# ArmastusChen/Learning-Continuous-Implicit-Representation-for-Near-Periodic-Patterns

Hardware: AMD Instinct MI355X
Metric: fitted pixels/sec/GPU (512^2 grid, 256-wide MLP) + iters-to-target-PSNR (higher is better)
Workload: dtype bf16

## Files before the change

### learning-continuous-implicit-representation-for-near-periodic-patterns_amd/csrc/npp_api.hip

```cpp
#include <math.h>
#include <stdarg.h>
#include <stdio.h>
#include <string.h>
#include <vector>

#include "npp_adam.h"
#include "npp_chain16.h"
#include "npp_stash_census.h"

namespace npp {

static thread_local char g_err[512] = "";

void set_error(const char* fmt, ...) {
  va_list ap;
  va_start(ap, fmt);
  vsnprintf(g_err, sizeof(g_err), fmt, ap);
  va_end(ap);
}

int check_launch(const char* what) {
  hipError_t e = hipGetLastError();
  if (e != hipSuccess) {
    set_error("%s: %s", what, hipGetErrorString(e));
// ... 165 lines not shown
#pragma unroll
  for (int e = 0; e < 4; ++e) {
    if (e < cnt) {
      if (n < d.n_out[l]) {
        const __bf16 w = (__bf16)pn[e];
        if (!fwd4) {
          const int64_t pf = fwd_pack_pos(d, l, n, k);
          if (pf >= 0) a.wf[pf] = w;
        }
        const int64_t pb = bwd_pack_pos(b, l, n, k);
        if (pb >= 0) a.wb[pb] = w;
      }
      if (++k == d.n_in[l]) { k = 0; ++n; }
      if (n >= d.n_out[l] && i + e + 1 >= d.b_off[l] + d.n_out[l]) {
        do { ++l; } while (l < kNumLayers && !d.present[l]);
        if (l >= kNumLayers) break;
        n = 0; k = 0;
      }
    }
  }
}

static uint16_t f32_to_bf16_host(float f) {
  uint32_t u;
  memcpy(&u, &f, 4);
  if ((u & 0x7fffffffu) > 0x7f800000u) return (uint16_t)((u >> 16) | 0x40);
  u += 0x7FFF + ((u >> 16) & 1);
  return (uint16_t)(u >> 16);
}

__global__ void selftest_kernel(float* out) {
  const int lane = threadIdx.x & 63;
  const int m = lane & 31, h = lane >> 5;
  bf16x8 a, b;
#pragma unroll
  for (int j = 0; j < 8; ++j) {
    const int k = 8 * h + j;
    a[j] = (__bf16)(float)(((m * 3 + k * 5) % 5) - 2);
    b[j] = (__bf16)(float)(((k * 7 + m * 2) % 4) - 1);
  }
  f32x16 acc = {};
  acc = mfma_bf16(a, b, acc);
#pragma unroll
  for (int r = 0; r < 16; ++r) out[acc_row(r, h) * 32 + m] = acc[r];
  f32x16 y = {};
#pragma unroll
  for (int s = 0; s < 2; ++s) {
    bf16x8 x = pack_acc(acc, s), a2;
#pragma unroll
    for (int j = 0; j < 8; ++j) {
      const int k = 16 * s + perm16(h, j);
      a2[j] = (__bf16)(float)(((m * 5 + k * 3) % 7) - 3);
    }
    y = mfma_bf16(a2, x, y);
  }
#pragma unroll
  for (int r = 0; r < 16; ++r) out[1024 + acc_row(r, h) * 32 + m] = y[r];

  __shared__ __attribute__((aligned(16))) char tile[16384];
  for (int u = lane; u < 1024; u += 64) {
    const int hh = u & 1, b = (u >> 1) & 31, bt = (u >> 6) & 1, ks = u >> 7;
    bf16x8 f;
#pragma unroll
    for (int j = 0; j < 8; ++j) {
      const int feat = 16 * ks + perm16(hh, j), row = bt * 32 + b;
      f[j] = (__bf16)(float)(((7 * feat + 3 * row) % 251) - 125);
    }
    *(bf16x8*)(tile + wfmt_unit(8, 0, ks, bt, b, hh)) = f;
  }
  __syncthreads();
  for (int tt = 0; tt < 4; ++tt)
    for (int t = 0; t < 4; ++t) {
      const bf16x8 f = wfrag_read(tile, wfrag_offset(tt, t, lane));
#pragma unroll
      for (int j = 0; j < 8; ++j) out[2048 + ((tt * 4 + t) * 64 + lane) * 8 + j] = (float)f[j];
    }
}

static int tune_env(const char* name, int dflt) {
  const char* e = getenv(name);
  return e && *e ? atoi(e) : dflt;
}
Tunables g_tune = {tune_env("NPP_CONV_WINK", 1), tune_env("NPP_CONV_WIN", 1), tune_env("NPP_CONV_WSTAT", 1), tune_env("NPP_CONV_PAIR", 15),
                   tune_env("NPP_LIGHT_DET", 1), tune_env("NPP_STASH8", 1)};

}

using namespace npp;

extern "C" {

int npp_version(void) { return 100; }

int npp_tune(const char* key, int value) {
  struct { const char* k; int* v; } tab[] = {{"conv_wink", &g_tune.conv_wink}, {"conv_win", &g_tune.conv_win},
                                             {"conv_wstat", &g_tune.conv_wstat}, {"conv_pair", &g_tune.conv_pair},
                                             {"stash8", &g_tune.stash8}, {"light_det", &g_tune.light_det}};
  if (key)
    for (auto& t : tab)
      if (!strcmp(key, t.k)) {
        const int old = __atomic_load_n(t.v, __ATOMIC_RELAXED);
        if (value >= 0) __atomic_store_n(t.v, value, __ATOMIC_RELAXED);
        return old;
      }
  set_error("npp_tune: unknown key '%s'", key ? key : "(null)");
  return NPP_ERR_ARG;
}
const char* npp_last_error_string(void) { return g_err; }

int npp_device_count(void) {
  int n = 0;
  hipError_t e = hipGetDeviceCount(&n);
  if (e != hipSuccess) {
    set_error("hipGetDeviceCount: %s", hipGetErrorString(e));
    (void)hipGetLastError();
    return 0;
  }
  return n;
}

static int check_kw(int K, int width) {
  if (K < 1 || K > NPP_MAX_K) { set_error("K=%d outside [1,%d]", K, NPP_MAX_K); return NPP_ERR_ARG; }
  if (width != NPP_WIDTH) {
    set_error("width=%d: this build is specialised for width %d", width, NPP_WIDTH);
    return NPP_ERR_UNSUPPORTED;
  }
  return NPP_OK;
}

int npp_param_layout(int K, int width, const char** names, int64_t* offsets, int32_t* rows,
                     int32_t* cols, int64_t* total) {
  int rc = check_kw(K, width);
  if (rc) return rc;
  const NetDesc d = make_desc(K);
  int n = 0;
  for (int l = 0; l < kNumLayers; ++l) {
    if (!d.present[l]) continue;
    for (int wb = 0; wb < 2; ++wb) {
      snprintf(g_name_buf[n], sizeof(g_name_buf[n]), "%s.%s", kNames[l], wb ? "bias" : "weight");
      if (names) names[n] = g_name_buf[n];
      if (offsets) offsets[n] = wb ? d.b_off[l] : d.w_off[l];
      if (rows) rows[n] = d.n_out[l];
      if (cols) cols[n] = wb ? 1 : d.n_in[l];
      ++n;
    }
  }
  if (total) *total = d.total_params;
  return n;
}

int64_t npp_pack_bytes(int K, int width, int which) {
  if (check_kw(K, width)) return -1;
  return 16 * (which == 0 ? make_desc(K).wf_total16 : bwd_total16(K));
}

int npp_pack_weights(const float* d_params, void* d_wf, void* d_wb, int K, int width, void* stream) {
  int rc = check_kw(K, width);
  if (rc) return rc;
  if (!d_params || !d_wf || !d_wb) { set_error("npp_pack_weights: null pointer"); return NPP_ERR_ARG; }
  const NetDesc d = make_desc(K);
  const BwdDesc b = make_bwd_desc(K);
  const int64_t nf = d.wf_total16, nb = bwd_total16(K);
  const int threads = 256;
  const int64_t blocks = (nf + nb + threads - 1) / threads;
  hipLaunchKernelGGL(pack_weights_kernel, dim3((unsigned)blocks), dim3(threads), 0, (hipStream_t)stream,
                     d_params, (bf16x8*)d_wf, (bf16x8*)d_wb, d, b, nf, nb);
  return check_launch("npp_pack_weights");
}

int npp_pack_weights_host(const float* params, void* wf, void* wb, int K, int width) {
  int rc = check_kw(K, width);
  if (rc) return rc;
  const NetDesc d = make_desc(K);
  const BwdDesc b = make_bwd_desc(K);
  uint16_t* f = (uint16_t*)wf;
  uint16_t* g = (uint16_t*)wb;
  for (int64_t u = 0; u < d.wf_total16; ++u) {
    int l, ks, nt, lane;
    if (!fwd_unit(d, u, l, ks, nt, lane)) { set_error("fwd unit %lld unmapped", (long long)u); return NPP_ERR_ARG; }
    for (int j = 0; j < 8; ++j) f[u * 8 + j] = f32_to_bf16_host(fwd_pack_value(params, d, l, ks, nt, lane, j));
// ... 242 lines not shown
```

### learning-continuous-implicit-representation-for-near-periodic-patterns_amd/csrc/npp_common.h

```cpp
#pragma once
#include <hip/hip_runtime.h>
#include <math.h>
#include <stdint.h>
#include "npp_layout.h"

typedef __attribute__((ext_vector_type(8))) __bf16 bf16x8;
typedef __attribute__((ext_vector_type(4))) __bf16 bf16x4;
typedef __attribute__((ext_vector_type(2))) __bf16 bf16x2;
typedef __attribute__((ext_vector_type(16))) float f32x16;
typedef __attribute__((ext_vector_type(4))) float f32x4;
typedef __attribute__((ext_vector_type(2))) float f32x2;
typedef __attribute__((ext_vector_type(4))) uint32_t u32x4;
typedef __attribute__((ext_vector_type(8))) _Float16 f16x8;

namespace npp {

void set_error(const char* fmt, ...);
int check_launch(const char* what);
struct SmemOnce { unsigned long long done = 0; };
bool smem_attr(SmemOnce& once, const void* fn, int bytes);

constexpr int kLdsDefault = 48 * 1024;
template <auto Kern, typename... Args>
int launch_lds(const char* who, dim3 grid, dim3 block, size_t lds_bytes, int lds_limit, hipStream_t stream, const Args&... args) {
  static SmemOnce once;
  if (lds_limit && !smem_attr(once, (const void*)Kern, lds_limit)) { set_error("%s: smem attribute", who); return NPP_ERR_LAUNCH; }
  hipLaunchKernelGGL(Kern, grid, block, lds_bytes, stream, args...);
  return check_launch(who);
}

struct Tunables {
  int conv_wink;
  int conv_win;
  int conv_wstat;
  int conv_pair;
  int light_det;
  int stash8;
};
extern Tunables g_tune;

constexpr float kInv2Pi = 0.15915494309189535f;

__device__ __forceinline__ float snake_fast(float z) {
  const float s = __builtin_amdgcn_sinf(z * kInv2Pi);
  return fmaf(s, s, z);
}
__device__ __forceinline__ void snake_fast2(float z, float& a, float& da) {
  const float rev = z * kInv2Pi;
  const float s = __builtin_amdgcn_sinf(rev);
  const float c = __builtin_amdgcn_cosf(rev);
  a = fmaf(s, s, z);
  da = fmaf(2.0f * s, c, 1.0f);
}

__device__ __forceinline__ void wg_barrier() {
  asm volatile("s_waitcnt lgkmcnt(0)" ::: "memory");
  __builtin_amdgcn_s_barrier();
  asm volatile("" ::: "memory");
}

using wrsrc_t = __amdgpu_buffer_rsrc_t;
__device__ __forceinline__ wrsrc_t make_wrsrc(const void* pack, int64_t units16) {
  return __builtin_amdgcn_make_buffer_rsrc(const_cast<void*>(pack), 0, (int)(units16 * 16), 0x00020000);
}

struct StackIter {
  int32_t active, k, comp, with_lp;
  int32_t x0, nk, same, pad1;
  float step_size, inv_sqrt_bc2, pad2, pad3;
};
static_assert(sizeof(StackIter) == 48, "npp_stack_iter layout");
struct Stack {
  int32_t M;
  int32_t g;
  int32_t n_items;
  int32_t pad;
  const StackIter* iter;
};
inline Stack make_stack(int M, int n_items, const void* d_iter) {
  Stack S{};
  S.M = M; S.n_items = n_items; S.iter = (const StackIter*)d_iter;
  S.g = (M == 1 || M == 2 || M == 4 || M == 8) ? 8 / M : 0;
  return S;
}
inline unsigned stack_grid(const Stack& S) {
  return S.g ? 8u * (unsigned)((S.n_items + S.g - 1) / S.g) : (unsigned)S.M * (unsigned)S.n_items;
}
__device__ __forceinline__ bool stack_decode(const Stack& S, int& img, int& item, int& xslot, int& xcount) {
  const int b = (int)blockIdx.x;
  if (S.M == 0) { img = 0; item = b; xslot = b >> 3; xcount = ((int)gridDim.x + 7) >> 3; return true; }
  if (S.g) {
    const int xcd = b & 7, slot = b >> 3;
    img = xcd / S.g;
    item = slot * S.g + xcd % S.g;
    xslot = slot; xcount = (S.n_items + S.g - 1) / S.g;
  } else {
    img = b / S.n_items;
    item = b - img * S.n_items;
    xslot = item >> 3; xcount = (S.n_items + 7) >> 3;
  }
  if (item >= S.n_items) return false;
  return S.iter == nullptr || S.iter[img].active != 0;
}

}
```

### learning-continuous-implicit-representation-for-near-periodic-patterns_amd/csrc/npp_cx.hip

```cpp
#include <stdlib.h>

#include "npp_robust.h"
#include <type_traits>
#include "npp_trunk_layout.h"

namespace npp {

__global__ void patch_gather_kernel(const float* __restrict__ img, const float* __restrict__ mask, int H, int W,
                                    const int32_t* __restrict__ centres, int M, int P, float* __restrict__ out_rgb,
                                    float* __restrict__ out_mask) {
  const int m = blockIdx.y;
  const int cy = centres[2 * m], cx = centres[2 * m + 1];
  for (int idx = blockIdx.x * blockDim.x + threadIdx.x; idx < P * P; idx += gridDim.x * blockDim.x) {
    const int py = idx / P, px = idx - py * P;
    const int y = cy - P / 2 + py, x = cx - P / 2 + px;
    const bool in = y >= 0 && y < H && x >= 0 && x < W;
    const int64_t src = (int64_t)y * W + x;
#pragma unroll
    for (int c = 0; c < 3; ++c) out_rgb[((int64_t)m * 3 + c) * P * P + idx] = in ? img[src * 3 + c] : 0.0f;
    if (out_mask) out_mask[(int64_t)m * P * P + idx] = in ? mask[src] : 0.0f;
  }
}

struct CxWs {
  float* mu;
  float* ssx;
  float* ssy;
  unsigned* dmin;
  float* s;
  unsigned* cmax;
  float* dot;
  float* g;
  float* lsum;
  unsigned* ticket;
  float* inx;
  float* iny;
  float* D;
  float* cx;
  const StackIter* iter;
  int32_t M, mu_stride, N, dot_slots;
  int32_t min_in_rows;
};
__device__ __forceinline__ int cx_group(const CxWs& w, int n, int& ng) {
  if (!w.iter) { ng = w.N; return 0; }
  int m = 0;
  for (int j = 1; j < w.M; ++j)
    if (w.iter[j].nk > 0 && n >= w.iter[j].x0) m = j;
  ng = w.iter[m].nk;
  return m;
}
__device__ __forceinline__ const float* cx_mu(const CxWs& w, int n) {
  int ng;
  return w.mu + (int64_t)cx_group(w, n, ng) * w.mu_stride;
}

__host__ __device__ inline int64_t cx_ws_floats(int N, int C, int hw) {
  return (int64_t)NPP_MAX_STACK * (C + 16) + (7LL + C / 32) * N * hw + 3LL * N + 2LL * N * hw * hw + 160;
}

__host__ inline CxWs carve(float* base, int N, int C, int hw, const void* iter = nullptr, int M = 0) {
  CxWs w;
  float* p = base;
  w.iter = (const StackIter*)iter; w.M = M; w.N = N; w.mu_stride = (C + 15) / 16 * 16; w.dot_slots = C / 32; w.min_in_rows = 0;
  w.mu = p; p += (int64_t)(M > 0 ? M : 1) * w.mu_stride;
  const int64_t nh = (int64_t)N * hw;
  w.ssx = p; p += nh;
  w.ssy = p; p += nh;
  w.dmin = (unsigned*)p; p += nh;
  w.s = p; p += nh;
  w.cmax = (unsigned*)p; p += nh;
  w.dot = p; p += nh * w.dot_slots;
  w.g = p; p += (N + 15) / 16 * 16;
  w.lsum = p; p += (N + 15) / 16 * 16;
  w.ticket = (unsigned*)p; p += (N + 1 + 15) / 16 * 16;
  w.inx = p; p += nh;
  w.iny = p; p += nh;
  w.D = p; p += nh * hw;
  w.cx = p;
  return w;
}

__device__ __forceinline__ float inv_norm(float ss) { return 1.0f / fmaxf(sqrtf(ss), 1e-12f); }

// ... 408 lines not shown
  }
}

constexpr int kBigR = 8;
__global__ __launch_bounds__(256) void cx_colmax_big_kernel(int N, int hw, float inv_h, CxWs w, const float* __restrict__ s4) {
  __shared__ float red[4][128];
  const int wave = threadIdx.x >> 6, lane = threadIdx.x & 63;
  const int tiles = (hw + 127) / 128;
  int b = blockIdx.x;
  const int rg = b % kBigR; b /= kBigR;
  const int tj = b % tiles, n = b / tiles;
  if (n >= N) return;
  const int tr = (tiles + kBigR - 1) / kBigR;
  float best0 = 0.0f, best1 = 0.0f;
  for (int ti = rg * tr; ti < min(tiles, (rg + 1) * tr); ++ti) {
    const float* Dt = w.D + (((int64_t)n * tiles + ti) * tiles + tj) * 16384 + wave * 128 + 2 * lane;
    const int irow = ti * 128 + wave + 4 * (lane & 31);
    float my_rdm = 0.0f, my_rs = 0.0f;
    if (irow < hw) {
      const int64_t row = (int64_t)n * hw + irow;
      my_rdm = 1.0f / (__uint_as_float(w.dmin[row]) + 1e-5f);
      const float* sq = s4 + row * kBigQ;
      my_rs = 1.0f / (((sq[0] + sq[1]) + sq[2]) + sq[3]);
    }
#pragma unroll
    for (int k = 0; k < 32; ++k) {
      const float2 d = *(const float2*)(Dt + k * 512);
      const float rdm = __shfl(my_rdm, k, 64), rs = __shfl(my_rs, k, 64);
      const float c0 = __expf((1.0f - d.x * rdm) * inv_h) * rs, c1 = __expf((1.0f - d.y * rdm) * inv_h) * rs;
      best0 = fmaxf(best0, rs > 0.0f ? c0 : 0.0f);
      best1 = fmaxf(best1, rs > 0.0f ? c1 : 0.0f);
    }
  }
  red[wave][2 * lane] = best0;
  red[wave][2 * lane + 1] = best1;
  __syncthreads();
  if (threadIdx.x < 128) {
    const int j = tj * 128 + threadIdx.x;
    const float v = fmaxf(fmaxf(red[0][threadIdx.x], red[1][threadIdx.x]), fmaxf(red[2][threadIdx.x], red[3][threadIdx.x]));
    if (j < hw) atomicMax(&w.cmax[(int64_t)n * hw + j], __float_as_uint(v));
  }
}

__global__ void cx_loss_kernel(int N, int hw, const float* __restrict__ weight, float scale, float* __restrict__ loss,
                               int loss_stride, CxWs w) {
  __shared__ float red[4];
  const int n = blockIdx.x;
  int ng;
  cx_group(w, n, ng);
  float acc = 0.0f;
  for (int j = threadIdx.x; j < hw; j += blockDim.x) {
    acc += __uint_as_float(w.cmax[(int64_t)n * hw + j]);
    w.inx[(int64_t)n * hw + j] = inv_norm(w.ssx[(int64_t)n * hw + j]);
    w.iny[(int64_t)n * hw + j] = inv_norm(w.ssy[(int64_t)n * hw + j]);
  }
  for (int off = 32; off > 0; off >>= 1) acc += __shfl_xor(acc, off, 64);
  if ((threadIdx.x & 63) == 0) red[threadIdx.x >> 6] = acc;
  __syncthreads();
  if (threadIdx.x == 0) {
    const float cxn = (red[0] + red[1] + red[2] + red[3]) / (float)hw;
    float l, dcxn;
    if (weight) {
      const float wt = weight[n];
      l = -logf(cxn * wt + 1e-5f);
      dcxn = -wt / (cxn * wt + 1e-5f);
    } else {
      l = -logf(cxn + 1e-5f) / (float)ng;
      dcxn = -1.0f / ((float)ng * (cxn + 1e-5f));
    }
    share_store(w.lsum + n, scale * l);
    w.g[n] = scale * dcxn / (float)hw;
  }
  if (!block_last_arriver(w.ticket, N)) return;
  const int groups = w.iter ? w.M : 1;
  if ((int)threadIdx.x < groups) {
    const int grp = threadIdx.x;
    const int n0 = w.iter ? w.iter[grp].x0 : 0, cnt = w.iter ? w.iter[grp].nk : N;
    float total = 0.0f;
    for (int q = n0; q < n0 + cnt; ++q) total += share_load(w.lsum + q);
    if (cnt > 0) atomicAdd(loss + (int64_t)grp * loss_stride, total);
  }
}

__global__ __launch_bounds__(256) void cx_rows_bwd_kernel(int N, int hw, float inv_h, CxWs w, float* __restrict__ loss, int loss_stride) {
  const int wave = threadIdx.x >> 6, lane = threadIdx.x & 63;
  if (loss && blockIdx.x == 0 && (int)threadIdx.x < (w.iter ? w.M : 1)) {
    const int grp = threadIdx.x;
    const int n0 = w.iter ? w.iter[grp].x0 : 0, cnt = w.iter ? w.iter[grp].nk : N;
    float total = 0.0f;
    for (int q = n0; q < n0 + cnt; ++q) total += w.lsum[q];
    if (cnt > 0) atomicAdd(loss + (int64_t)grp * loss_stride, total);
  }
  const int64_t row = (int64_t)blockIdx.x * 4 + wave;
  if (row >= (int64_t)N * hw) return;
  const int n = (int)(row / hw);
  const float dmv = __uint_as_float(w.dmin[row]);
  const float dm = dmv + 1e-5f;
  const float s = w.s[row], g = w.g[n];
  const float* Dr = w.D + row * hw;
  float* cr = w.cx + row * hw;
  const unsigned* cm = w.cmax + (int64_t)n * hw;
  float A = 0.0f;
  for (int j = lane; j < hw; j += 64) {
    const float c = cr[j];
    if (__float_as_uint(c) == cm[j]) A += g * c;
  }
  for (int off = 32; off > 0; off >>= 1) A += __shfl_xor(A, off, 64);
  float corr = 0.0f;
  int jmin = 0x7fffffff;
  for (int j = lane; j < hw; j += 64) {
    const float c = cr[j], d = Dr[j];
    const float G = (__float_as_uint(c) == cm[j]) ? g : 0.0f;
    const float wv = c * s;
    const float dDt = -((G - A) / s) * wv * inv_h;
    corr += dDt * d;
    const float dD = dDt / dm;
    cr[j] = (d > 0.0f && d < 1.0f) ? -dD : 0.0f;
    if (d == dmv) jmin = min(jmin, j);
  }
  for (int off = 32; off > 0; off >>= 1) {
    corr += __shfl_xor(corr, off, 64);
    jmin = min(jmin, __shfl_xor(jmin, off, 64));
  }
  if (jmin < hw && lane == (jmin & 63)) {
    const float d = Dr[jmin];
    if (d > 0.0f && d < 1.0f) cr[jmin] += corr / (dm * dm);
  }
}

__global__ __launch_bounds__(256) void cx_dx_kernel(const float* __restrict__ x, const float* __restrict__ y, int N, int C,
                                                    int hw, CxWs w, float* __restrict__ dxh) {
  __shared__ float sA[2][kCxKc][65];
  __shared__ float sB[2][kCxKc][65];
  const int tid = threadIdx.x, wave = tid >> 6, lane = tid & 63;
  const int itiles = (hw + 63) / 64, ctiles = (C + 63) / 64;
  const int n = blockIdx.x / (ctiles * itiles);
  const int rem = blockIdx.x - n * ctiles * itiles;
  const int c0 = (rem / itiles) * 64, i0 = (rem % itiles) * 64;
  const int wc = wave >> 1, wi = wave & 1, l31 = lane & 31, kh = lane >> 5;
  const bool vec = (hw & 3) == 0;
  const float* iny_ss = w.ssy + (int64_t)n * hw;
  const float* mup = cx_mu(w, n);
  float4 ra[2], rb[2];
  auto gload = [&](int j0) {
#pragma unroll
    for (int r = 0; r < 2; ++r) {
      const int idx = tid + 256 * r, row = idx >> 3, col = (idx & 7) * 4;
      const int j = j0 + col;
      float va[4] = {0, 0, 0, 0}, vb[4] = {0, 0, 0, 0};
      const int c = c0 + row, i = i0 + row;
      if (c < C) {
        const float m = mup[c];
        const float* yr = y + ((int64_t)n * C + c) * hw;
        if (vec && j + 3 < hw) { const float4 q = *(const float4*)(yr + j); va[0] = q.x - m; va[1] = q.y - m; va[2] = q.z - m; va[3] = q.w - m; }
        else for (int e = 0; e < 4; ++e) if (j + e < hw) va[e] = yr[j + e] - m;
        for (int e = 0; e < 4; ++e) va[e] = (j + e < hw) ? va[e] * inv_norm(iny_ss[j + e]) : 0.0f;
      }
      if (i < hw) {
        const float* dr = w.cx + ((int64_t)n * hw + i) * hw;
        if (vec && j + 3 < hw) { const float4 q = *(const float4*)(dr + j); vb[0] = q.x; vb[1] = q.y; vb[2] = q.z; vb[3] = q.w; }
        else for (int e = 0; e < 4; ++e) if (j + e < hw) vb[e] = dr[j + e];
      }
      ra[r] = make_float4(va[0], va[1], va[2], va[3]);
      rb[r] = make_float4(vb[0], vb[1], vb[2], vb[3]);
    }
  };
  auto sstore = [&](int buf) {
#pragma unroll
    for (int r = 0; r < 2; ++r) {
      const int idx = tid + 256 * r, row = idx >> 3, col = (idx & 7) * 4;
      sA[buf][col + 0][row] = ra[r].x; sA[buf][col + 1][row] = ra[r].y; sA[buf][col + 2][row] = ra[r].z; sA[buf][col + 3][row] = ra[r].w;
      sB[buf][col + 0][row] = rb[r].x; sB[buf][col + 1][row] = rb[r].y; sB[buf][col + 2][row] = rb[r].z; sB[buf][col + 3][row] = rb[r].w;
    }
  };
  f32x16 acc;
#pragma unroll
  for (int r = 0; r < 16; ++r) acc[r] = 0.0f;
  gload(0);
  sstore(0);
  __syncthreads();
  int buf = 0;
  for (int j0 = 0; j0 < hw; j0 += kCxKc) {
    const bool has_next = j0 + kCxKc < hw;
    if (has_next) gload(j0 + kCxKc);
#pragma unroll
    for (int ks = 0; ks < kCxKc / 2; ++ks) {
      const float a = sA[buf][2 * ks + kh][wc * 32 + l31];
      const float b = sB[buf][2 * ks + kh][wi * 32 + l31];
      acc = __builtin_amdgcn_mfma_f32_32x32x2f32(a, b, acc, 0, 0, 0);
    }
    if (has_next) sstore(buf ^ 1);
    __syncthreads();
    buf ^= 1;
  }
  const int i = i0 + wi * 32 + l31;
  float part = 0.0f;
  if (i < hw) {
    const float inx = inv_norm(w.ssx[(int64_t)n * hw + i]);
#pragma unroll
    for (int r = 0; r < 16; ++r) {
      const int c = c0 + wc * 32 + acc_row(r, kh);
      if (c < C) {
        const int64_t o = ((int64_t)n * C + c) * hw + i;
        dxh[o] = acc[r];
        part = fmaf((x[o] - mup[c]) * inx, acc[r], part);
      }
    }
  }
  part += __shfl_xor(part, 32, 64);
  const int slot = c0 / 32 + wc;
  if (kh == 0 && i < hw && slot < w.dot_slots) w.dot[(int64_t)slot * N * hw + (int64_t)n * hw + i] = part;
}

__global__ void cx_dx_finish_kernel(const float* __restrict__ x, int N, int C, int hw, CxWs w, float* __restrict__ dx, int n_dot) {
  const int64_t t = (int64_t)blockIdx.x * blockDim.x + threadIdx.x;
  if (t >= (int64_t)N * C * hw) return;
  const int p = (int)(t % hw);
  const int64_t nc = t / hw;
  const int c = (int)(nc % C), n = (int)(nc / C);
  const float inx = inv_norm(w.ssx[(int64_t)n * hw + p]);
  float dot = 0.0f;
  for (int q = 0; q < n_dot; ++q) dot += w.dot[(int64_t)q * N * hw + (int64_t)n * hw + p];
  dx[t] = (dx[t] - (x[t] - cx_mu(w, n)[c]) * inx * dot) * inx;
}

__global__ void cx_dx_finish_flat_kernel(const float* __restrict__ x, const float* __restrict__ dxh, int N, int N_total, int C, int H,
                                         int W, CxWs w, const f16x8* __restrict__ yact, bf16x8* __restrict__ dz, int64_t nposp,
                                         int64_t npos_range, int n_dot) {
  const int64_t t = (int64_t)blockIdx.x * blockDim.x + threadIdx.x;
  const int chunks = C / 8;
  if (t >= npos_range * chunks) return;
  const int c8 = (int)(t / npos_range);
  const int64_t p = t - (int64_t)c8 * npos_range;
  const int Wp = W + 2, S = (H + 2) * Wp, hw = H * W;
  const int n = (int)(p / S), r = (int)(p - (int64_t)n * S), yy = r / Wp, xx = r - yy * Wp;
  if (n >= N && n < N_total) return;
  const int64_t u = (int64_t)c8 * nposp + kConvGuard + p;
  bf16x8 o;
#pragma unroll
  for (int j = 0; j < 8; ++j) o[j] = (__bf16)0.0f;
  if (n < N && yy >= 1 && yy <= H && xx >= 1 && xx <= W) {
    const int pos = (yy - 1) * W + (xx - 1);
    const int64_t np = (int64_t)n * hw + pos;
    const float inx = inv_norm(w.ssx[np]);
    float dot = 0.0f;
    for (int q = 0; q < n_dot; ++q) dot += w.dot[(int64_t)q * N * hw + np];
    const float* mu = cx_mu(w, n);
    const f16x8 m = yact[u];
#pragma unroll
    for (int j = 0; j < 8; ++j) {
      const int c = conv_chan(c8, j);
      const int64_t e = ((int64_t)n * C + c) * hw + pos;
      const float v = (dxh[e] - (x[e] - mu[c]) * inx * dot) * inx;
      o[j] = (__bf16)((float)m[j] > 0.0f ? v : 0.0f);
    }
  }
  dz[u] = o;
}


constexpr int kDxLd = 33;
__global__ __launch_bounds__(256) void cx_dx32s_kernel(const float* __restrict__ x, const float* __restrict__ y, int N, int C,
                                                       int hw, CxWs w, float* __restrict__ dxh) {
  __shared__ float sY[2][4][32][kDxLd];
  __shared__ float sD[2][32][kDxLd];
  const int tid = threadIdx.x, wave = tid >> 6, lane = tid & 63, l31 = lane & 31, kh = lane >> 5;
  const int t32 = hw / 32, ct = C / 32, cg = ct / 4 + (ct % 4 ? 1 : 0);
  const int lb = xcd_block(N * t32 * cg);
  if (lb < 0) return;
  const int n = lb / (t32 * cg);
  const int rem = lb - n * t32 * cg;
  const int ti = rem / cg, tc0 = (rem - ti * cg) * 4, tc = tc0 + wave;
  const int i0 = ti * 32, c0 = tc * 32;
  const float* mup = cx_mu(w, n);
  const int srow = tid >> 3, scol = tid & 7;
  const float4* dsrc = (const float4*)(w.cx + ((int64_t)n * hw + i0 + srow) * hw) + scol;
  const float4* ssrc = (const float4*)(w.iny + (int64_t)n * hw) + scol;
  const float4* ysrc[4];
  float mus[4];
#pragma unroll
  for (int q = 0; q < 4; ++q) {
    const int c = (tc0 + q) * 32 + srow;
    const bool ok = c < C;
    ysrc[q] = (const float4*)(y + ((int64_t)n * C + (ok ? c : 0)) * hw) + scol;
    mus[q] = ok ? mup[c] : 0.0f;
  }
  struct Raw { float4 d, s, yv[4]; };
  Raw R;
  auto gissue = [&](int jb) {
    R.d = dsrc[8 * jb];
    R.s = ssrc[8 * jb];
#pragma unroll
    for (int q = 0; q < 4; ++q) R.yv[q] = ysrc[q][8 * jb];
  };
  auto sstore = [&](int buf) {
    const int k0 = 4 * scol;
    sD[buf][k0 + 0][srow] = R.d.x; sD[buf][k0 + 1][srow] = R.d.y; sD[buf][k0 + 2][srow] = R.d.z; sD[buf][k0 + 3][srow] = R.d.w;
#pragma unroll
    for (int q = 0; q < 4; ++q) {
      const float m = mus[q];
      sY[buf][q][k0 + 0][srow] = (R.yv[q].x - m) * R.s.x; sY[buf][q][k0 + 1][srow] = (R.yv[q].y - m) * R.s.y;
      sY[buf][q][k0 + 2][srow] = (R.yv[q].z - m) * R.s.z; sY[buf][q][k0 + 3][srow] = (R.yv[q].w - m) * R.s.w;
    }
  };
  f32x16 acc;
#pragma unroll
  for (int r = 0; r < 16; ++r) acc[r] = 0.0f;
  const int nblk = hw / 32;
  gissue(0);
  sstore(0);
  __syncthreads();
  int buf = 0;
  for (int jb = 0; jb < nblk; ++jb) {
    const bool has_next = jb + 1 < nblk;
    if (has_next) gissue(jb + 1);
#pragma unroll
    for (int t = 0; t < 4; ++t)
#pragma unroll
      for (int e = 0; e < 4; ++e) {
        const int k = 8 * t + 4 * kh + e;
        acc = __builtin_amdgcn_mfma_f32_32x32x2f32(sY[buf][wave][k][l31], sD[buf][k][l31], acc, 0, 0, 0);
      }
    if (has_next) sstore(buf ^ 1);
    __syncthreads();
    buf ^= 1;
  }
  if (tc >= ct) return;
  const int i = i0 + l31;
  const float inx = w.inx[(int64_t)n * hw + i];
  float part = 0.0f;
#pragma unroll
  for (int r = 0; r < 16; ++r) {
    const int c = c0 + acc_row(r, kh);
    const int64_t o = ((int64_t)n * C + c) * hw + i;
    dxh[o] = acc[r];
    part = fmaf((x[o] - mup[c]) * inx, acc[r], part);
  }
  part += __shfl_xor(part, 32, 64);
  if (kh == 0) w.dot[(int64_t)tc * N * hw + (int64_t)n * hw + i] = part;
}

constexpr int kCxRowsPerWave = 1;
constexpr int kCxRowWaves = 16;
__global__ __launch_bounds__(64 * kCxRowWaves) void cx_rows_fwd32_kernel(int N, int hw, float inv_h, CxWs w, float scale, int with_loss) {
  extern __shared__ float scm[];
  const int wave = threadIdx.x >> 6, lane = threadIdx.x & 63;
  const int blocks_per_n = (hw + kCxRowWaves * kCxRowsPerWave - 1) / (kCxRowWaves * kCxRowsPerWave);
  const int n = blockIdx.x / blocks_per_n;
  const int r0 = (blockIdx.x - n * blocks_per_n) * kCxRowWaves * kCxRowsPerWave + wave * kCxRowsPerWave;
  float cmaxv[kCxMaxCols];
#pragma unroll
  for (int q = 0; q < kCxMaxCols; ++q) cmaxv[q] = 0.0f;
  const int ncol = (hw + 63) / 64;
  for (int rr = 0; rr < kCxRowsPerWave; ++rr) {
    if (r0 + rr >= hw) break;
    const int64_t row = (int64_t)n * hw + r0 + rr;
    const float* Dr = w.D + row * hw;
    float* cr = w.cx + row * hw;
    float wv[kCxMaxCols];
    float s = 0.0f;
    float dm;
    if (w.min_in_rows) {
      float mn = 2.0f;
#pragma unroll
      for (int q = 0; q < kCxMaxCols; ++q) {
        if (q < ncol) {
          const int j = lane + 64 * q;
          wv[q] = j < hw ? Dr[j] : 2.0f;
          mn = fminf(mn, wv[q]);
        }
      }
      for (int off = 32; off > 0; off >>= 1) mn = fminf(mn, __shfl_xor(mn, off, 64));
      if (lane == 0) w.dmin[row] = __float_as_uint(mn);
      dm = mn + 1e-5f;
#pragma unroll
      for (int q = 0; q < kCxMaxCols; ++q) {
        if (q < ncol) {
          const int j = lane + 64 * q;
          wv[q] = j < hw ? __expf((1.0f - wv[q] / dm) * inv_h) : 0.0f;
          s += wv[q];
        }
      }
    } else {
      dm = __uint_as_float(w.dmin[row]) + 1e-5f;
#pragma unroll
      for (int q = 0; q < kCxMaxCols; ++q) {
        if (q < ncol) {
          const int j = lane + 64 * q;
          wv[q] = j < hw ? __expf((1.0f - Dr[j] / dm) * inv_h) : 0.0f;
          s += wv[q];
        }
      }
    }
    for (int off = 32; off > 0; off >>= 1) s += __shfl_xor(s, off, 64);
    if (lane == 0) w.s[row] = s;
    const float inv = 1.0f / s;
#pragma unroll
    for (int q = 0; q < kCxMaxCols; ++q) {
      if (q < ncol) {
        const int j = lane + 64 * q;
        if (j < hw) {
          const float c = wv[q] * inv;
          cr[j] = c;
          cmaxv[q] = fmaxf(cmaxv[q], c);
        }
      }
    }
  }
#pragma unroll
  for (int q = 0; q < kCxMaxCols; ++q) {
    if (q < ncol) {
      const int j = lane + 64 * q;
      if (j < hw) scm[wave * hw + j] = cmaxv[q];
    }
  }
  __syncthreads();
  for (int j = threadIdx.x; j < hw; j += 64 * kCxRowWaves) {
    float m = scm[j];
#pragma unroll
    for (int v = 1; v < kCxRowWaves; ++v) m = fmaxf(m, scm[v * hw + j]);
    atomicMax(&w.cmax[(int64_t)n * hw + j], __float_as_uint(m));
  }
// ... 20 lines not shown
    w.g[n] = scale * (-1.0f / ((float)ng * (cxn + 1e-5f))) / (float)hw;
  }
}

}

using namespace npp;

extern "C" int npp_patch_gather(const float* d_img_hwc, const float* d_mask_hw, int H, int W, const int32_t* d_centres_yx,
                                int M, int P, float* d_out_rgb, float* d_out_mask, void* stream) {
  if (!d_img_hwc || !d_centres_yx || !d_out_rgb || H < 1 || W < 1 || M < 0 || P < 2 || (P & 1)) {
    set_error("npp_patch_gather: bad arguments (M=%d, P=%d must be even)", M, P);
    return NPP_ERR_ARG;
  }
  if (d_out_mask && !d_mask_hw) { set_error("npp_patch_gather: out_mask without mask"); return NPP_ERR_ARG; }
  if (M == 0) return NPP_OK;
  const int bx = (P * P + 255) / 256;
  hipLaunchKernelGGL(patch_gather_kernel, dim3(bx, M), dim3(256), 0, (hipStream_t)stream, d_img_hwc, d_mask_hw, H, W,
                     d_centres_yx, M, P, d_out_rgb, d_out_mask);
  return check_launch("npp_patch_gather");
}

extern "C" int64_t npp_cx_workspace_bytes(int N, int C, int hw) {
  if (N < 1 || C < 32 || (C % 32) || hw < 1) { set_error("npp_cx_workspace_bytes: need N>=1, C multiple of 32, hw>=1"); return -1; }
  return 4 * cx_ws_floats(N, C, hw);
}

struct CxFlatOut {
  const void* yact;
  void* dz;
  int N_total, H, W;
};
static bool big_fwd_fits(int N, int C, int hw) {
  const int64_t t = (hw + 127) / 128;
  return (int64_t)N * (t * t * 16384 + 2 * t * C * 128 + (int64_t)hw * kBigQ) <= 2LL * N * hw * hw;
}
static int cx_launch(const float* d_fx, const float* d_fy, int N, int C, int hw, float band_width, const float* d_weight,
                     float scale, float* d_loss, int loss_stride, float* d_dfx, void* d_workspace, int64_t workspace_bytes,
                     const void* d_iter, int M, void* stream, const char* who, const CxFlatOut* flat = nullptr) {
  if (!d_fx || !d_fy || !d_loss || !d_workspace || N < 1 || C < 32 || (C % 32) || hw < 1 || !(band_width > 0.0f) ||
      (int64_t)N * hw * hw > 0x7fffffffLL * 8 || M < 0 || M > NPP_MAX_STACK || (M > 0 && !d_iter)) {
    set_error("%s: bad arguments (N=%d C=%d hw=%d M=%d)", who, N, C, hw, M);
    return NPP_ERR_ARG;
  }
  if (workspace_bytes < 4 * cx_ws_floats(N, C, hw)) { set_error("%s: workspace too small", who); return NPP_ERR_ARG; }
  hipStream_t s = (hipStream_t)stream;
  CxWs w = carve((float*)d_workspace, N, C, hw, d_iter, M);
  const int groups = M > 0 ? M : 1;
  const int64_t nh = (int64_t)N * hw;
  const float inv_h = 1.0f / band_width;
  const bool big = hw > 64 * kCxMaxCols;
  const bool fast = !big && (hw % 32) == 0;
  w.min_in_rows = fast ? 1 : 0;
  hipLaunchKernelGGL(cx_mean_kernel, dim3(C, groups), dim3(256), 0, s, d_fy, N, C, hw, w);
  const int tiles = (hw + 63) / 64;
  const bool loss_in_rows = fast && d_dfx && !d_weight;
  const int t32 = hw / 32;
  if (fast) {
    hipLaunchKernelGGL(cx_sim_kernel, dim3((unsigned)(((int64_t)N * tiles * tiles + 7) / 8 * 8)), dim3(256), 0, s, d_fx, d_fy, N, C, hw, w);
    const size_t smem = (size_t)kCxRowWaves * hw * sizeof(float);
    constexpr int kRowLdsMax = kCxRowWaves * 64 * kCxMaxCols * 4;
    const int rc = launch_lds<cx_rows_fwd32_kernel>(who, dim3((unsigned)((int64_t)N * ((hw + kCxRowWaves - 1) / kCxRowWaves))), dim3(64 * kCxRowWaves), smem,
                                                    smem > (size_t)kLdsDefault ? kRowLdsMax : 0, s, N, hw, inv_h, w, scale, (int)loss_in_rows);
    if (rc) return rc;
  } else if (big && !d_dfx && big_fwd_fits(N, C, hw)) {
    const int t128 = (hw + 127) / 128;
    const int64_t t8 = (t128 + 7) / 8;
    if ((int64_t)N * t8 * t8 * 64 > 0x7fffffffLL) { set_error("%s: grid too large", who); return NPP_ERR_ARG; }
    float* xt = w.D + (int64_t)N * t128 * t128 * 16384;
    float* yt = xt + (int64_t)N * t128 * C * 128;
    float* s4 = yt + (int64_t)N * t128 * C * 128;
    hipLaunchKernelGGL(cx_prep_big_kernel, dim3((unsigned)(2 * N * t128)), dim3(256), 0, s, d_fx, d_fy, N, C, hw, w, xt, yt);
    hipLaunchKernelGGL(cx_sim_big_kernel, dim3((unsigned)((int64_t)N * t8 * t8 * 64)), dim3(256), 0, s, xt, yt, N, C, hw, w);
    hipLaunchKernelGGL(cx_rowsum_big_kernel, dim3((unsigned)(N * t128 * kBigQ)), dim3(256), 0, s, N, hw, inv_h, w, s4);
    hipLaunchKernelGGL(cx_colmax_big_kernel, dim3((unsigned)(N * t128 * kBigR)), dim3(256), 0, s, N, hw, inv_h, w, s4);
  } else {
    hipLaunchKernelGGL(cx_sim_kernel, dim3((unsigned)(((int64_t)N * tiles * tiles + 7) / 8 * 8)), dim3(256), 0, s, d_fx, d_fy, N, C, hw, w);
    const int64_t row_groups = (int64_t)N * ((hw + kCxRows - 1) / kCxRows);
    if (big) hipLaunchKernelGGL(cx_rows_fwd_big_kernel, dim3((unsigned)((row_groups + 3) / 4)), dim3(256), 0, s, N, hw, inv_h, w);
    else hipLaunchKernelGGL(cx_rows_fwd_kernel, dim3((unsigned)((row_groups + 3) / 4)), dim3(256), 0, s, N, hw, inv_h, w);
  }
  if (!loss_in_rows) hipLaunchKernelGGL(cx_loss_kernel, dim3(N), dim3(256), 0, s, N, hw, d_weight, scale, d_loss, loss_stride, w);
  if (d_dfx) {
    hipLaunchKernelGGL(cx_rows_bwd_kernel, dim3((unsigned)((nh + 3) / 4)), dim3(256), 0, s, N, hw, inv_h, w, loss_in_rows ? d_loss : nullptr,
                       loss_stride);
    const int ctiles = (C + 63) / 64;
    if (fast) {
      const int64_t nb_dx = (int64_t)N * t32 * ((C / 32 + 3) / 4);
      hipLaunchKernelGGL(cx_dx32s_kernel, dim3((unsigned)((nb_dx + 7) / 8 * 8)), dim3(256), 0, s, d_fx, d_fy, N, C, hw, w, d_dfx);
    }
    else
      hipLaunchKernelGGL(cx_dx_kernel, dim3((unsigned)((int64_t)N * ctiles * tiles)), dim3(256), 0, s, d_fx, d_fy, N, C, hw, w,
                         d_dfx);
    if (flat) {
      if (!flat->yact || !flat->dz || flat->H * flat->W != hw || N > flat->N_total || C % 16) {
        set_error("%s: bad flat-output description", who); return NPP_ERR_ARG;
      }
      const int64_t range = conv_npos_round(N, flat->H, flat->W), nt = range * (C / 8);
      hipLaunchKernelGGL(cx_dx_finish_flat_kernel, dim3((unsigned)((nt + 255) / 256)), dim3(256), 0, s, d_fx, d_dfx, N, flat->N_total, C, flat->H,
                         flat->W, w, (const f16x8*)flat->yact, (bf16x8*)flat->dz, conv_nposp(flat->N_total, flat->H, flat->W), range, C / 32);
      return check_launch(who);
    }
    const int64_t ne = nh * C;
    hipLaunchKernelGGL(cx_dx_finish_kernel, dim3((unsigned)((ne + 255) / 256)), dim3(256), 0, s, d_fx, N, C, hw, w, d_dfx, C / 32);
  }
  return check_launch(who);
}

extern "C" int npp_cx_fwd_bwd(const float* d_fx, const float* d_fy, int N, int C, int hw, float band_width,
                              const float* d_weight, float scale, float* d_loss, float* d_dfx, void* d_workspace,
                              int64_t workspace_bytes, void* stream) {
  return cx_launch(d_fx, d_fy, N, C, hw, band_width, d_weight, scale, d_loss, 0, d_dfx, d_workspace, workspace_bytes, nullptr, 0,
                   stream, "npp_cx_fwd_bwd");
}

extern "C" int npp_cx_fwd_bwd_groups(const float* d_fx, const float* d_fy, int N, int C, int hw, float band_width, float scale,
                                     float* d_loss, int loss_stride, float* d_dfx, const void* d_iter, int M, void* d_workspace,
                                     int64_t workspace_bytes, void* stream) {
  if (M < 1) { set_error("npp_cx_fwd_bwd_groups: M=%d", M); return NPP_ERR_ARG; }
  return cx_launch(d_fx, d_fy, N, C, hw, band_width, nullptr, scale, d_loss, loss_stride, d_dfx, d_workspace, workspace_bytes, d_iter,
                   M, stream, "npp_cx_fwd_bwd_groups");
}

extern "C" int npp_cx_fwd_bwd_flat(const float* d_fx, const float* d_fy, int N, int C, int H, int W, float band_width, float scale,
                                   float* d_loss, int loss_stride, float* d_scratch_dfx, const void* d_yact, void* d_dz, int N_total,
                                   const void* d_iter, int M, void* d_workspace, int64_t workspace_bytes, void* stream) {
  if (!d_scratch_dfx) { set_error("npp_cx_fwd_bwd_flat: null scratch"); return NPP_ERR_ARG; }
  const CxFlatOut flat{d_yact, d_dz, N_total, H, W};
  return cx_launch(d_fx, d_fy, N, C, H * W, band_width, nullptr, scale, d_loss, loss_stride, d_scratch_dfx, d_workspace, workspace_bytes,
                   d_iter, M, stream, "npp_cx_fwd_bwd_flat", &flat);
}
```

Before: 46.02 million.

## Fuse CX backward dx contraction with finish via precomputed row dot products

Computes the per-row normalization dot product inside cx_rows_bwd_kernel (using dr*(1-d)) so the dx32 contraction kernel can apply the final normalization and ReLU-masked bf16 flat output directly. This removes the separate finish kernel and the intermediate dxh round trip through global memory. Extra trailing blocks zero the padding/halo of the flat output. It is enabled by default via a new cx_fused tunable, and it relies on the algebraic identity for the dot term matching the old channel-wise reduction.

```diff
diff --git a/learning-continuous-implicit-representation-for-near-periodic-patterns_amd/csrc/npp_api.hip b/learning-continuous-implicit-representation-for-near-periodic-patterns_amd/csrc/npp_api.hip
--- a/learning-continuous-implicit-representation-for-near-periodic-patterns_amd/csrc/npp_api.hip
+++ b/learning-continuous-implicit-representation-for-near-periodic-patterns_amd/csrc/npp_api.hip
@@ -271,7 +271,7 @@
   return e && *e ? atoi(e) : dflt;
 }
 Tunables g_tune = {tune_env("NPP_CONV_WINK", 1), tune_env("NPP_CONV_WIN", 1), tune_env("NPP_CONV_WSTAT", 1), tune_env("NPP_CONV_PAIR", 15),
-                   tune_env("NPP_LIGHT_DET", 1), tune_env("NPP_STASH8", 1)};
+                   tune_env("NPP_LIGHT_DET", 1), tune_env("NPP_STASH8", 1), tune_env("NPP_CX_FUSED", 1)};
 
 }
 
@@ -284,7 +284,8 @@
 int npp_tune(const char* key, int value) {
   struct { const char* k; int* v; } tab[] = {{"conv_wink", &g_tune.conv_wink}, {"conv_win", &g_tune.conv_win},
                                              {"conv_wstat", &g_tune.conv_wstat}, {"conv_pair", &g_tune.conv_pair},
-                                             {"stash8", &g_tune.stash8}, {"light_det", &g_tune.light_det}};
+                                             {"stash8", &g_tune.stash8}, {"light_det", &g_tune.light_det},
+                                             {"cx_fused", &g_tune.cx_fused}};
   if (key)
     for (auto& t : tab)
       if (!strcmp(key, t.k)) {
diff --git a/learning-continuous-implicit-representation-for-near-periodic-patterns_amd/csrc/npp_common.h b/learning-continuous-implicit-representation-for-near-periodic-patterns_amd/csrc/npp_common.h
--- a/learning-continuous-implicit-representation-for-near-periodic-patterns_amd/csrc/npp_common.h
+++ b/learning-continuous-implicit-representation-for-near-periodic-patterns_amd/csrc/npp_common.h
@@ -36,6 +36,7 @@
   int conv_pair;
   int light_det;
   int stash8;
+  int cx_fused;
 };
 extern Tunables g_tune;
 
diff --git a/learning-continuous-implicit-representation-for-near-periodic-patterns_amd/csrc/npp_cx.hip b/learning-continuous-implicit-representation-for-near-periodic-patterns_amd/csrc/npp_cx.hip
--- a/learning-continuous-implicit-representation-for-near-periodic-patterns_amd/csrc/npp_cx.hip
+++ b/learning-continuous-implicit-representation-for-near-periodic-patterns_amd/csrc/npp_cx.hip
@@ -1,4 +1,5 @@
 #include <stdlib.h>
+#include <algorithm>
 
 #include "npp_robust.h"
 #include <type_traits>
@@ -573,7 +574,8 @@
   }
 }
 
-__global__ __launch_bounds__(256) void cx_rows_bwd_kernel(int N, int hw, float inv_h, CxWs w, float* __restrict__ loss, int loss_stride) {
+__global__ __launch_bounds__(256) void cx_rows_bwd_kernel(int N, int hw, float inv_h, CxWs w, float* __restrict__ loss, int loss_stride,
+                                                          float* __restrict__ dot_out) {
   const int wave = threadIdx.x >> 6, lane = threadIdx.x & 63;
   if (loss && blockIdx.x == 0 && (int)threadIdx.x < (w.iter ? w.M : 1)) {
     const int grp = threadIdx.x;
@@ -597,7 +599,7 @@
     if (__float_as_uint(c) == cm[j]) A += g * c;
   }
   for (int off = 32; off > 0; off >>= 1) A += __shfl_xor(A, off, 64);
-  float corr = 0.0f;
+  float corr = 0.0f, dot = 0.0f;
   int jmin = 0x7fffffff;
   for (int j = lane; j < hw; j += 64) {
     const float c = cr[j], d = Dr[j];
@@ -606,16 +608,26 @@
     const float dDt = -((G - A) / s) * wv * inv_h;
     corr += dDt * d;
     const float dD = dDt / dm;
-    cr[j] = (d > 0.0f && d < 1.0f) ? -dD : 0.0f;
+    const float dr = (d > 0.0f && d < 1.0f) ? -dD : 0.0f;
+    cr[j] = dr;
+    dot += dr * (1.0f - d);
     if (d == dmv) jmin = min(jmin, j);
   }
   for (int off = 32; off > 0; off >>= 1) {
     corr += __shfl_xor(corr, off, 64);
+    dot += __shfl_xor(dot, off, 64);
     jmin = min(jmin, __shfl_xor(jmin, off, 64));
   }
-  if (jmin < hw && lane == (jmin & 63)) {
-    const float d = Dr[jmin];
-    if (d > 0.0f && d < 1.0f) cr[jmin] += corr / (dm * dm);
+  if (lane == (jmin < hw ? (jmin & 63) : 0)) {
+    if (jmin < hw) {
+      const float d = Dr[jmin];
+      if (d > 0.0f && d < 1.0f) {
+        const float fix = corr / (dm * dm);
+        cr[jmin] += fix;
+        dot += fix * (1.0f - d);
+      }
+    }
+    if (dot_out) dot_out[row] = dot;
   }
 }
 
@@ -751,18 +763,16 @@
 
 
 constexpr int kDxLd = 33;
-__global__ __launch_bounds__(256) void cx_dx32s_kernel(const float* __restrict__ x, const float* __restrict__ y, int N, int C,
-                                                       int hw, CxWs w, float* __restrict__ dxh) {
+struct Dx32Tile { int n, i0, tc, ct; };
+__device__ __forceinline__ Dx32Tile cx_dx32_contract(const float* __restrict__ y, int N, int C, int hw, const CxWs& w, int lb, f32x16& acc) {
   __shared__ float sY[2][4][32][kDxLd];
   __shared__ float sD[2][32][kDxLd];
   const int tid = threadIdx.x, wave = tid >> 6, lane = tid & 63, l31 = lane & 31, kh = lane >> 5;
   const int t32 = hw / 32, ct = C / 32, cg = ct / 4 + (ct % 4 ? 1 : 0);
-  const int lb = xcd_block(N * t32 * cg);
-  if (lb < 0) return;
   const int n = lb / (t32 * cg);
   const int rem = lb - n * t32 * cg;
-  const int ti = rem / cg, tc0 = (rem - ti * cg) * 4, tc = tc0 + wave;
-  const int i0 = ti * 32, c0 = tc * 32;
+  const int ti = rem / cg, tc0 = (rem - ti * cg) * 4;
+  const int i0 = ti * 32;
   const float* mup = cx_mu(w, n);
   const int srow = tid >> 3, scol = tid & 7;
   const float4* dsrc = (const float4*)(w.cx + ((int64_t)n * hw + i0 + srow) * hw) + scol;
@@ -794,7 +804,6 @@
       sY[buf][q][k0 + 2][srow] = (R.yv[q].z - m) * R.s.z; sY[buf][q][k0 + 3][srow] = (R.yv[q].w - m) * R.s.w;
     }
   };
-  f32x16 acc;
 #pragma unroll
   for (int r = 0; r < 16; ++r) acc[r] = 0.0f;
   const int nblk = hw / 32;
@@ -816,19 +825,96 @@
     __syncthreads();
     buf ^= 1;
   }
-  if (tc >= ct) return;
-  const int i = i0 + l31;
+  return Dx32Tile{n, i0, tc0 + wave, ct};
+}
+
+__global__ __launch_bounds__(256) void cx_dx32s_kernel(const float* __restrict__ x, const float* __restrict__ y, int N, int C,
+                                                       int hw, CxWs w, float* __restrict__ dxh) {
+  const int t32 = hw / 32, ct = C / 32, cg = ct / 4 + (ct % 4 ? 1 : 0);
+  const int lb = xcd_block(N * t32 * cg);
+  if (lb < 0) return;
+  f32x16 acc;
+  const Dx32Tile T = cx_dx32_contract(y, N, C, hw, w, lb, acc);
+  if (T.tc >= T.ct) return;
+  const int l31 = threadIdx.x & 31, kh = (threadIdx.x >> 5) & 1, n = T.n;
+  const float* mup = cx_mu(w, n);
+  const int i = T.i0 + l31;
   const float inx = w.inx[(int64_t)n * hw + i];
   float part = 0.0f;
 #pragma unroll
   for (int r = 0; r < 16; ++r) {
-    const int c = c0 + acc_row(r, kh);
+    const int c = T.tc * 32 + acc_row(r, kh);
     const int64_t o = ((int64_t)n * C + c) * hw + i;
     dxh[o] = acc[r];
     part = fmaf((x[o] - mup[c]) * inx, acc[r], part);
   }
   part += __shfl_xor(part, 32, 64);
-  if (kh == 0) w.dot[(int64_t)tc * N * hw + (int64_t)n * hw + i] = part;
+  if (kh == 0) w.dot[(int64_t)T.tc * N * hw + (int64_t)n * hw + i] = part;
+}
+
+__device__ __forceinline__ float cx_finish(float dxh, float x, float mu, float inx, float dot) { return (dxh - (x - mu) * inx * dot) * inx; }
+
+struct CxFlatDev {
+  const f16x8* yact;
+  bf16x8* dz;
+  int64_t nposp, range;
+  int N_total, H, W;
+};
+template <bool FLAT>
+__global__ __launch_bounds__(256) void cx_dx32f_kernel(const float* __restrict__ x, const float* __restrict__ y, int N, int C, int hw,
+                                                       CxWs w, float* __restrict__ dfx, CxFlatDev f, int nb) {
+  const int g0 = (nb + 7) / 8 * 8;
+  int lb = blockIdx.x;
+  if (lb < g0) lb = (lb & 7) * (g0 >> 3) + (lb >> 3);
+  if (lb >= nb) {
+    if constexpr (FLAT) {
+      const int Wp = f.W + 2, S = (f.H + 2) * Wp;
+      const int64_t total = f.range * (C / 8), step = (int64_t)(gridDim.x - nb) * 256;
+      bf16x8 z;
+#pragma unroll
+      for (int j = 0; j < 8; ++j) z[j] = (__bf16)0.0f;
+      for (int64_t t = (int64_t)(lb - nb) * 256 + threadIdx.x; t < total; t += step) {
+        const int c8 = (int)(t / f.range);
+        const int64_t p = t - (int64_t)c8 * f.range;
+        const int n = (int)(p / S), r = (int)(p - (int64_t)n * S), yy = r / Wp, xx = r - yy * Wp;
+        if (n >= N && n < f.N_total) continue;
+        if (n < N && yy >= 1 && yy <= f.H && xx >= 1 && xx <= f.W) continue;
+        f.dz[(int64_t)c8 * f.nposp + kConvGuard + p] = z;
+      }
+    }
+    return;
+  }
+  f32x16 acc;
+  const Dx32Tile T = cx_dx32_contract(y, N, C, hw, w, lb, acc);
+  if (T.tc >= T.ct) return;
+  const int l31 = threadIdx.x & 31, kh = (threadIdx.x >> 5) & 1, n = T.n;
+  const float* mup = cx_mu(w, n);
+  const int i = T.i0 + l31;
+  const float inx = w.inx[(int64_t)n * hw + i], dot = w.dot[(int64_t)n * hw + i];
+  if constexpr (FLAT) {
+    const int Wp = f.W + 2, py = i / f.W, px = i - py * f.W;
+    const int64_t p = (int64_t)n * (f.H + 2) * Wp + (py + 1) * Wp + px + 1;
+#pragma unroll
+    for (int half = 0; half < 2; ++half) {
+      const int64_t u = (int64_t)(4 * T.tc + 2 * half + kh) * f.nposp + kConvGuard + p;
+      const f16x8 m = f.yact[u];
+      bf16x8 o;
+#pragma unroll
+      for (int j = 0; j < 8; ++j) {
+        const int c = T.tc * 32 + acc_row(8 * half + j, kh);
+        const float v = cx_finish(acc[8 * half + j], x[((int64_t)n * C + c) * hw + i], mup[c], inx, dot);
+        o[j] = (__bf16)((float)m[j] > 0.0f ? v : 0.0f);
+      }
+      f.dz[u] = o;
+    }
+  } else {
+#pragma unroll
+    for (int r = 0; r < 16; ++r) {
+      const int c = T.tc * 32 + acc_row(r, kh);
+      const int64_t o = ((int64_t)n * C + c) * hw + i;
+      dfx[o] = cx_finish(acc[r], x[o], mup[c], inx, dot);
+    }
+  }
 }
 
 constexpr int kCxRowsPerWave = 1;
@@ -1015,20 +1101,35 @@
   }
   if (!loss_in_rows) hipLaunchKernelGGL(cx_loss_kernel, dim3(N), dim3(256), 0, s, N, hw, d_weight, scale, d_loss, loss_stride, w);
   if (d_dfx) {
+    if (flat && (!flat->yact || !flat->dz || flat->H * flat->W != hw || N > flat->N_total || C % 16)) {
+      set_error("%s: bad flat-output description", who); return NPP_ERR_ARG;
+    }
+    const bool fused = fast && __atomic_load_n(&g_tune.cx_fused, __ATOMIC_RELAXED) != 0;
     hipLaunchKernelGGL(cx_rows_bwd_kernel, dim3((unsigned)((nh + 3) / 4)), dim3(256), 0, s, N, hw, inv_h, w, loss_in_rows ? d_loss : nullptr,
-                       loss_stride);
+                       loss_stride, fused ? w.dot : nullptr);
     const int ctiles = (C + 63) / 64;
+    const int64_t nb_dx = (int64_t)N * t32 * ((C / 32 + 3) / 4);
+    if (fused) {
+      if (nb_dx + 256 + 8 > 0x7fffffffLL) { set_error("%s: grid too large", who); return NPP_ERR_ARG; }
+      const int64_t g0 = (nb_dx + 7) / 8 * 8;
+      if (flat) {
+        CxFlatDev f{(const f16x8*)flat->yact, (bf16x8*)flat->dz, conv_nposp(flat->N_total, flat->H, flat->W), conv_npos_round(N, flat->H, flat->W),
+                    flat->N_total, flat->H, flat->W};
+        const int64_t nz = std::min<int64_t>(256, (f.range * (C / 8) + 1023) / 1024);
+        hipLaunchKernelGGL(cx_dx32f_kernel<true>, dim3((unsigned)std::max(g0, nb_dx + nz)), dim3(256), 0, s, d_fx, d_fy, N, C, hw, w,
+                           (float*)nullptr, f, (int)nb_dx);
+      } else {
+        hipLaunchKernelGGL(cx_dx32f_kernel<false>, dim3((unsigned)g0), dim3(256), 0, s, d_fx, d_fy, N, C, hw, w, d_dfx, CxFlatDev{}, (int)nb_dx);
+      }
+      return check_launch(who);
+    }
     if (fast) {
-      const int64_t nb_dx = (int64_t)N * t32 * ((C / 32 + 3) / 4);
       hipLaunchKernelGGL(cx_dx32s_kernel, dim3((unsigned)((nb_dx + 7) / 8 * 8)), dim3(256), 0, s, d_fx, d_fy, N, C, hw, w, d_dfx);
     }
     else
       hipLaunchKernelGGL(cx_dx_kernel, dim3((unsigned)((int64_t)N * ctiles * tiles)), dim3(256), 0, s, d_fx, d_fy, N, C, hw, w,
                          d_dfx);
     if (flat) {
-      if (!flat->yact || !flat->dz || flat->H * flat->W != hw || N > flat->N_total || C % 16) {
-        set_error("%s: bad flat-output description", who); return NPP_ERR_ARG;
-      }
       const int64_t range = conv_npos_round(N, flat->H, flat->W), nt = range * (C / 8);
       hipLaunchKernelGGL(cx_dx_finish_flat_kernel, dim3((unsigned)((nt + 255) / 256)), dim3(256), 0, s, d_fx, d_dfx, N, flat->N_total, C, flat->H,
                          flat->W, w, (const f16x8*)flat->yact, (bf16x8*)flat->dz, conv_nposp(flat->N_total, flat->H, flat->W), range, C / 32);
```

New measurement: 46.47 million (median of 6 runs). Within noise of the previous version (+1.0%).
